# lab-emi/CleanUMamba

Measured on AMD Instinct MI355X. Metric: audio samples/sec/node (train step, E8, 10s@16kHz), higher is better.
Workload: dtype f16; 1 GPU; CleanUMamba-E8 (41.4M) full train step: fwd + L1 + multi-res STFT loss + bwd + grad all-reduce + clip + Adam; 10 s @ 16 kHz clips; global_batch=16, batch_per_gpu=16, clip_samples=160000, parallelism=dp1, weights=random init (reference init, seed 0)

## Files before the change

cleanumamba_amd/csrc/dec7.hip:

```cpp
#include "outer_common.h"

namespace cum {

constexpr int D7_H = 64;
constexpr int D7_J = 128;
constexpr int D7_R = 32;
constexpr int D7_ZS = 288;
constexpr int D7_US = 144;
constexpr int D7_SLAB = D7_J * D7_H + D7_J + D7_H * 4 + 2;

struct Dec7FwdParams {
  const void *u;
  const void *w1p;
  const float *b1p;
  const float *wt;
  const float *bt;
  void *out;
  int64_t M;
  int pitch, valid;
  int64_t zero_tail;
  int steps_per_wg;
};

template <typename T>
__global__ __launch_bounds__(256) void dec7_fwd_kernel(const Dec7FwdParams p) {
  static_assert(sizeof(T) == 2, "16-bit element types only");
  __shared__ __attribute__((aligned(16))) unsigned char ut_all[2][D7_R * D7_US];
  __shared__ float4 pv_all[2][4][D7_R];
  __shared__ float carry[2][2];

  const int tid = threadIdx.x, lane = tid & 63;
  const int w = uniform(tid >> 6);
  const int g = lane >> 4, r = lane & 15;
  const T *u = static_cast<const T *>(p.u) + D7_H;
  T *out = static_cast<T *>(p.out) + 8;
  if (blockIdx.x == 0) {
    if (tid < 8) out[tid - 8] = (T)0.f;
    for (int64_t i = tid; i < p.zero_tail; i += 256) out[2 * p.M * 8 + i] = (T)0.f;
  }
// ... 82 lines not shown
        }
      }
      if (row == 0) {
        prv[2] = carry[par ^ 1][0];
        prv[3] = carry[par ^ 1][1];
      }
      if (row == D7_R - 1) carry[par][q] = cur[2 + q];
      const int64_t m = m0 + row;
      if (s >= s_begin && m < p.M) {
        const bool ok = e0_row_ok(t0, row, m0, p.M, (unsigned)p.pitch, (unsigned)p.valid + 1u);
        const float v = ok ? cur[q] + prv[2 + q] + btv : 0.f;
        *reinterpret_cast<uint4 *>(out + (2 * m + q) * 8) = make_uint4(e0_pack2<T>(v, 0.f), 0u, 0u, 0u);
      }
    }
  }
}

struct Dec7BwdParams {
  const void *u;
  const void *dy;
  const unsigned char *mask;
  const void *w1p;
  const float *b1p;
  const float *wt;
  void *du;
  void *dpre;
  float *slabs;
  int64_t M;
  int pitch, valid;
  int64_t zero_tail;
};

template <typename T>
__global__ __launch_bounds__(256) void dec7_bwd_kernel(const Dec7BwdParams p) {
  static_assert(sizeof(T) == 2, "16-bit element types only");
  constexpr int BUF = D7_R * D7_US + D7_R * D7_ZS + 2 * D7_R * D7_US + 320 + 512;
  __shared__ __attribute__((aligned(16))) unsigned char lds[2 * BUF];

  const int tid = threadIdx.x, lane = tid & 63;
  const int w = uniform(tid >> 6);
  const int g = lane >> 4, r = lane & 15;
  const T *u = static_cast<const T *>(p.u) + D7_H;
  const T *dy = static_cast<const T *>(p.dy);
  T *du = static_cast<T *>(p.du) + D7_H, *dpre = static_cast<T *>(p.dpre) + D7_H;
  if (blockIdx.x == 0) {
    for (int i = tid; i < D7_H; i += 256) du[i - D7_H] = dpre[i - D7_H] = (T)0.f;
    for (int64_t i = tid; i < p.zero_tail; i += 256) du[p.M * D7_H + i] = dpre[p.M * D7_H + i] = (T)0.f;
  }
  e0_u32x4 wA[2][2], wB[4];
  float ba[4], bb[4], wtr[4][4];
  {
    const T *w1 = static_cast<const T *>(p.w1p);
#pragma unroll
    for (int jt = 0; jt < 2; ++jt)
#pragma unroll
      for (int ks = 0; ks < 2; ++ks)
        wA[jt][ks] = *reinterpret_cast<const e0_u32x4 *>(w1 + (int64_t)(32 * w + 16 * jt + r) * D7_H + 32 * ks + 8 * g);
#pragma unroll
    for (int ks = 0; ks < 4; ++ks) {
      unsigned v[4];
#pragma unroll
      for (int q = 0; q < 4; ++q) {
        const int j = 32 * ks + 8 * g + 2 * q;
        const unsigned short lo = __builtin_bit_cast(unsigned short, w1[(int64_t)j * D7_H + 16 * w + r]);
        const unsigned short hi = __builtin_bit_cast(unsigned short, w1[(int64_t)(j + 1) * D7_H + 16 * w + r]);
        v[q] = (unsigned)lo | ((unsigned)hi << 16);
      }
      wB[ks] = e0_u32x4{v[0], v[1], v[2], v[3]};
    }
#pragma unroll
    for (int rr = 0; rr < 4; ++rr) {
      ba[rr] = p.b1p[32 * w + 4 * g + rr];
      bb[rr] = p.b1p[32 * w + 16 + 4 * g + rr];
#pragma unroll
      for (int k = 0; k < 4; ++k) wtr[rr][k] = (float)(T)p.wt[(16 * w + 4 * g + rr) * 4 + k];
    }
  }
  const unsigned one2 = __is_same(T, f16) ? 0x3C003C00u : 0x3F803F80u;
  const e0_u32x4 ones = e0_u32x4{one2, one2, one2, one2};

  e0_f32x4 acc1[2][4];
  e0_f32x4 accb[2];
#pragma unroll
  for (int it = 0; it < 2; ++it) {
    accb[it] = e0_f32x4{0.f, 0.f, 0.f, 0.f};
#pragma unroll
    for (int nt = 0; nt < 4; ++nt) acc1[it][nt] = e0_f32x4{0.f, 0.f, 0.f, 0.f};
  }
  float awt[4][4];
#pragma unroll
  for (int rr = 0; rr < 4; ++rr)
#pragma unroll
    for (int k = 0; k < 4; ++k) awt[rr][k] = 0.f;
  float sdy = 0.f;

  const int64_t nsteps = (p.M + D7_R - 1) / D7_R;
  constexpr int PF = 3;
  uint4 uc[PF];
  float xs[PF];
  unsigned mk[PF];
  auto fetch = [&](int64_t s, uint4 &c, float &x, unsigned &mw) {
    const int64_t m0 = s * D7_R;
    int64_t m = m0 + (tid >> 3);
    m = m < p.M ? m : p.M - 1;
    c = *reinterpret_cast<const uint4 *>(u + m * D7_H + (tid & 7) * 8);
    x = 0.f;
    if (tid < 72) {
      int64_t row = 1 + 2 * m0 + tid;
      const int64_t last = 2 * p.M + 2;
      row = row < last ? row : last;
      x = (float)dy[row * 8];
    }
    mw = 0u;
    if (tid >= 128) {
      int64_t mm = m0 + ((tid - 128) >> 2);
      mm = mm < p.M ? mm : p.M - 1;
      mw = *reinterpret_cast<const unsigned *>(p.mask + mm * 16 + (tid & 3) * 4);
    }
  };
  int64_t s = blockIdx.x;
#pragma unroll
  for (int i = 0; i < PF; ++i) {
    const int64_t sf = s + (int64_t)i * gridDim.x;
    fetch(sf < nsteps ? sf : nsteps - 1, uc[i], xs[i], mk[i]);
  }
  int par = 0;
  for (; s < nsteps; s += gridDim.x, par ^= 1) {
    unsigned char *ut = lds + par * BUF, *zt = ut + D7_R * D7_US, *dut = zt + D7_R * D7_ZS, *dpt = dut + D7_R * D7_US;
    float *xt = reinterpret_cast<float *>(dpt + D7_R * D7_US);
    unsigned *mt_ = reinterpret_cast<unsigned *>(xt + 80);
    const int64_t m0 = s * D7_R;
    const unsigned t0 = (unsigned)uniform((int)((unsigned)m0 % (unsigned)p.pitch));
    *reinterpret_cast<uint4 *>(ut + (tid >> 3) * D7_US + (tid & 7) * 16) = uc[0];
    if (tid < 72) xt[tid] = 2 * m0 + tid < 2 * p.M ? xs[0] : 0.f;
    if (tid >= 128) mt_[tid - 128] = mk[0];
    __syncthreads();
    {
#pragma unroll
      for (int i = 0; i + 1 < PF; ++i) {
        uc[i] = uc[i + 1];
        xs[i] = xs[i + 1];
        mk[i] = mk[i + 1];
      }
      const int64_t sf = s + (int64_t)PF * gridDim.x;
      if (sf < nsteps) fetch(sf, uc[PF - 1], xs[PF - 1], mk[PF - 1]);
    }
    if (w == 0) sdy += xt[lane];
#pragma unroll
    for (int mt = 0; mt < 2; ++mt) {
      e0_f32x4 da = e0_f32x4{0.f, 0.f, 0.f, 0.f}, db = da;
#pragma unroll
      for (int ks = 0; ks < 2; ++ks) {
        const e0_u32x4 ub = *reinterpret_cast<const e0_u32x4 *>(ut + (16 * mt + r) * D7_US + (4 * ks + g) * 16);
        da = e0_mfma<T>(wA[0][ks], ub, da);
        db = e0_mfma<T>(wA[1][ks], ub, db);
      }
      const int row = 16 * mt + r;
      const bool ok = e0_row_ok(t0, row, m0, p.M, (unsigned)p.pitch, (unsigned)p.valid);
      const float d0 = xt[2 * row], d1 = xt[2 * row + 1], d2 = xt[2 * row + 2], d3 = xt[2 * row + 3];
      float za[4], zb[4];
#pragma unroll
      for (int rr = 0; rr < 4; ++rr) {
        const float sg = sigmoidf_(db[rr] + bb[rr]);
        const float gv = e0_keep(ok, (float)(T)((da[rr] + ba[rr]) * sg));
        float dg = d0 * wtr[rr][0];
        dg = fmaf(d1, wtr[rr][1], dg);
        dg = fmaf(d2, wtr[rr][2], dg);
        dg = fmaf(d3, wtr[rr][3], dg);
        za[rr] = e0_keep(ok, dg * sg);
        zb[rr] = dg * gv * (1.f - sg);
        awt[rr][0] = fmaf(gv, d0, awt[rr][0]);
        awt[rr][1] = fmaf(gv, d1, awt[rr][1]);
        awt[rr][2] = fmaf(gv, d2, awt[rr][2]);
        awt[rr][3] = fmaf(gv, d3, awt[rr][3]);
      }
      *reinterpret_cast<uint2 *>(zt + row * D7_ZS + (32 * w + 4 * g) * 2) = make_uint2(e0_pack2<T>(za[0], za[1]), e0_pack2<T>(za[2], za[3]));
      *reinterpret_cast<uint2 *>(zt + row * D7_ZS + (32 * w + 16 + 4 * g) * 2) = make_uint2(e0_pack2<T>(zb[0], zb[1]), e0_pack2<T>(zb[2], zb[3]));
    }
    __syncthreads();
    {
      e0_f32x4 d1[2] = {e0_f32x4{0.f, 0.f, 0.f, 0.f}, e0_f32x4{0.f, 0.f, 0.f, 0.f}};
#pragma unroll
      for (int mt = 0; mt < 2; ++mt)
#pragma unroll
        for (int ks = 0; ks < 4; ++ks) {
          const e0_u32x4 a = *reinterpret_cast<const e0_u32x4 *>(zt + (16 * mt + r) * D7_ZS + (4 * ks + g) * 16);
          d1[mt] = e0_mfma<T>(a, wB[ks], d1[mt]);
        }
      const int h = 16 * w + r;
#pragma unroll
      for (int mt = 0; mt < 2; ++mt)
#pragma unroll
        for (int rr = 0; rr < 4; ++rr) {
          const int row = 16 * mt + 4 * g + rr;
          const unsigned bit = (reinterpret_cast<const unsigned char *>(mt_)[row * 16 + (h >> 2)] >> (h & 3)) & 1u;
          const T v = (T)d1[mt][rr];
          *reinterpret_cast<T *>(dut + row * D7_US + h * 2) = v;
          *reinterpret_cast<T *>(dpt + row * D7_US + h * 2) = bit ? v : (T)0.f;
        }
    }
    {
      const int q = r >> 2, pp = r & 3;
      e0_u32x4 af[2], bf[4];
#pragma unroll
      for (int it = 0; it < 2; ++it) af[it] = e0_tr_read<D7_ZS>(zt + (8 * g + q) * D7_ZS + (32 * w + 16 * it + 4 * pp) * 2);
#pragma unroll
      for (int nt = 0; nt < 4; ++nt) bf[nt] = e0_tr_read<D7_US>(ut + (8 * g + q) * D7_US + (16 * nt + 4 * pp) * 2);
#pragma unroll
      for (int it = 0; it < 2; ++it) {
#pragma unroll
        for (int nt = 0; nt < 4; ++nt) acc1[it][nt] = e0_mfma<T>(af[it], bf[nt], acc1[it][nt]);
        accb[it] = e0_mfma<T>(af[it], ones, accb[it]);
      }
    }
    __syncthreads();
    {
      const int row = tid >> 3, ch = tid & 7;
      const int64_t m = m0 + row;
      if (m < p.M) {
        *reinterpret_cast<uint4 *>(du + m * D7_H + ch * 8) = *reinterpret_cast<const uint4 *>(dut + row * D7_US + ch * 16);
        *reinterpret_cast<uint4 *>(dpre + m * D7_H + ch * 8) = *reinterpret_cast<const uint4 *>(dpt + row * D7_US + ch * 16);
      }
    }
  }

  float *slab = p.slabs + (int64_t)blockIdx.x * D7_SLAB;
#pragma unroll
  for (int it = 0; it < 2; ++it)
#pragma unroll
    for (int rr = 0; rr < 4; ++rr) {
      const int j = 32 * w + 16 * it + 4 * g + rr;
#pragma unroll
      for (int nt = 0; nt < 4; ++nt) slab[j * D7_H + 16 * nt + r] = acc1[it][nt][rr];
      if (r == 0) slab[D7_J * D7_H + j] = accb[it][rr];
    }
  float *s1 = slab + D7_J * D7_H + D7_J;
#pragma unroll
  for (int rr = 0; rr < 4; ++rr)
#pragma unroll
    for (int k = 0; k < 4; ++k) {
      const float v = row16_allsum(awt[rr][k]);
      if (r == 0) s1[(16 * w + 4 * g + rr) * 4 + k] = v;
    }
  if (w == 0) {
    sdy += __shfl_xor(sdy, 2, 64);
    sdy += __shfl_xor(sdy, 4, 64);
    sdy += __shfl_xor(sdy, 8, 64);
    sdy += __shfl_xor(sdy, 16, 64);
    sdy += __shfl_xor(sdy, 32, 64);
    if (lane < 2) s1[D7_H * 4 + lane] = sdy;
// ... 46 lines not shown
}

using namespace cum;

static int dec7_fwd_workgroups(int64_t M) {
  const int64_t steps = (M + D7_R - 1) / D7_R;
  return (int)(steps < 1024 ? steps : 1024);
}

extern "C" int cum_dec7_fwd(int32_t dtype, int64_t M, int32_t pitch, int32_t valid, const void *u, const void *w1p,
                            const float *b1p, const float *wt, const float *bt, void *out, int64_t zero_tail, void *stream) {
  CUM_REQUIRE(is16(dtype), "dec7_fwd: 16-bit element types only (f32 takes the generic path)");
  CUM_REQUIRE(M > 0 && M < 1073741823LL && pitch >= 32 && valid > 0 && valid < pitch && zero_tail >= 0, "dec7_fwd: bad geometry");
  CUM_REQUIRE(u && w1p && b1p && wt && bt && out, "dec7_fwd: null tensor");
  CUM_REQUIRE(((uintptr_t)u & 15) == 0 && ((uintptr_t)out & 15) == 0 && ((uintptr_t)w1p & 15) == 0,
              "dec7_fwd: u, out and w1p must be 16-byte aligned");
  hipStream_t st = (hipStream_t)stream;
  Dec7FwdParams p{};
  p.u = u; p.w1p = w1p; p.b1p = b1p; p.wt = wt; p.bt = bt; p.out = out; p.M = M; p.pitch = pitch; p.valid = valid;
  p.zero_tail = zero_tail;
  const int64_t steps = (M + D7_R - 1) / D7_R;
  int nwg = dec7_fwd_workgroups(M);
  p.steps_per_wg = (int)((steps + nwg - 1) / nwg);
  nwg = (int)((steps + p.steps_per_wg - 1) / p.steps_per_wg);
  if (dtype == CUM_F16)
    hipLaunchKernelGGL(dec7_fwd_kernel<f16>, dim3(nwg), dim3(256), 0, st, p);
  else
    hipLaunchKernelGGL(dec7_fwd_kernel<__bf16>, dim3(nwg), dim3(256), 0, st, p);
  CUM_CHECK_LAUNCH();
  return CUM_OK;
}

extern "C" int32_t cum_dec7_bwd_workgroups(int64_t M) {
  const int64_t steps = (M + D7_R - 1) / D7_R;
  return (int32_t)(steps < 1 ? 1 : (steps > 512 ? 512 : steps));
}

extern "C" int64_t cum_dec7_bwd_workspace_elems(int64_t M) {
  return ((int64_t)cum_dec7_bwd_workgroups(M) + D7_RG) * D7_SLAB;
}

extern "C" int cum_dec7_bwd(int32_t dtype, int64_t M, int32_t pitch, int32_t valid, const void *dY, const void *u,
                            const void *mask, const void *w1p, const float *b1p, const float *wt, void *dU, void *dpre,
                            int64_t zero_tail, float *slot_w1, float *slot_wt, float *workspace, void *stream) {
  CUM_REQUIRE(is16(dtype), "dec7_bwd: 16-bit element types only (f32 takes the generic path)");
  CUM_REQUIRE(M > 0 && M < 1073741823LL && pitch >= 32 && valid > 0 && valid < pitch && zero_tail >= 0, "dec7_bwd: bad geometry");
  CUM_REQUIRE(dY && u && mask && w1p && b1p && wt && dU && dpre && slot_w1 && slot_wt && workspace, "dec7_bwd: null tensor");
  CUM_REQUIRE(((uintptr_t)u & 15) == 0 && ((uintptr_t)dU & 15) == 0 && ((uintptr_t)dpre & 15) == 0 && ((uintptr_t)w1p & 15) == 0 &&
                  ((uintptr_t)mask & 3) == 0, "dec7_bwd: u, dU, dpre and w1p must be 16-byte aligned, mask 4-byte aligned");
  hipStream_t st = (hipStream_t)stream;
  Dec7BwdParams p{};
  p.u = u; p.dy = dY; p.mask = static_cast<const unsigned char *>(mask); p.w1p = w1p; p.b1p = b1p; p.wt = wt; p.du = dU;
  p.dpre = dpre; p.slabs = workspace; p.M = M; p.pitch = pitch; p.valid = valid; p.zero_tail = zero_tail;
  const int nwg = cum_dec7_bwd_workgroups(M);
  if (dtype == CUM_F16)
    hipLaunchKernelGGL(dec7_bwd_kernel<f16>, dim3(nwg), dim3(256), 0, st, p);
  else
    hipLaunchKernelGGL(dec7_bwd_kernel<__bf16>, dim3(nwg), dim3(256), 0, st, p);
  CUM_CHECK_LAUNCH();
  float *part = workspace + (int64_t)nwg * D7_SLAB;
  hipLaunchKernelGGL(dec7_bwd_reduce1_kernel, dim3((D7_SLAB + 255) / 256, D7_RG), dim3(256), 0, st, workspace, nwg, part);
  constexpr int nout = D7_J * D7_H + D7_J + 16 * 128 + 16;
  hipLaunchKernelGGL(dec7_bwd_reduce2_kernel, dim3((nout + 255) / 256), dim3(256), 0, st, part, slot_w1, slot_wt);
  CUM_CHECK_LAUNCH();
  return CUM_OK;
}
```

cleanumamba_amd/csrc/enc0.hip:

```cpp
#include "outer_common.h"

namespace cum {

constexpr int E0_H = 64;
constexpr int E0_J = 128;
constexpr int E0_R = 32;
constexpr int E0_ZS = 288;
constexpr int E0_YS = 144;
constexpr int E0_SLAB = E0_J * E0_H + E0_J + E0_H * 4 + E0_H;

struct Enc0BwdParams {
  const void *dz;
  const void *xin;
  const float *w1;
  const float *b1;
  const void *w2p;
  float *slabs;
  int64_t M;
  int pitch, valid;
};

template <typename T>
__global__ __launch_bounds__(256) void enc0_bwd_kernel(const Enc0BwdParams p) {
  static_assert(sizeof(T) == 2, "16-bit element types only");
// ... 16 lines not shown
  }
  e0_u32x4 wB[4];
  {
    const T *w2 = static_cast<const T *>(p.w2p);
#pragma unroll
    for (int ks = 0; ks < 4; ++ks) {
      unsigned v[4];
#pragma unroll
      for (int q = 0; q < 4; ++q) {
        const int j = 32 * ks + 8 * g + 2 * q;
        const unsigned short lo = __builtin_bit_cast(unsigned short, w2[(int64_t)j * E0_H + 16 * w + r]);
        const unsigned short hi = __builtin_bit_cast(unsigned short, w2[(int64_t)(j + 1) * E0_H + 16 * w + r]);
        v[q] = (unsigned)lo | ((unsigned)hi << 16);
      }
      wB[ks] = e0_u32x4{v[0], v[1], v[2], v[3]};
    }
  }
  const unsigned one2 = __is_same(T, f16) ? 0x3C003C00u : 0x3F803F80u;
  const e0_u32x4 ones = e0_u32x4{one2, one2, one2, one2};

  e0_f32x4 acc2[2][4];
  e0_f32x4 accb[2];
#pragma unroll
  for (int it = 0; it < 2; ++it) {
    accb[it] = e0_f32x4{0.f, 0.f, 0.f, 0.f};
#pragma unroll
    for (int nt = 0; nt < 4; ++nt) acc2[it][nt] = e0_f32x4{0.f, 0.f, 0.f, 0.f};
  }
  float a1[4] = {0.f, 0.f, 0.f, 0.f}, ab1 = 0.f;

  const int64_t nsteps = (p.M + E0_R - 1) / E0_R;
  constexpr int PF = 3;
  uint4 zc[PF][2];
  float xs[PF];
  auto fetch = [&](int64_t s, uint4 (&z)[2], float &x) {
    const int64_t m0 = s * E0_R;
#pragma unroll
    for (int it = 0; it < 2; ++it) {
      const int c = tid + 256 * it;
      int64_t m = m0 + (c >> 4);
      m = m < p.M ? m : p.M - 1;
      z[it] = *reinterpret_cast<const uint4 *>(dz + m * E0_J + (c & 15) * 8);
    }
    x = 0.f;
    if (tid < 72) {
      int64_t row = 1 + 2 * m0 + tid;
      const int64_t last = 2 * p.M + 2;
      row = row < last ? row : last;
      x = (float)xin[row * 8];
    }
  };
  int64_t s = blockIdx.x;
#pragma unroll
  for (int i = 0; i < PF; ++i) {
    const int64_t sf = s + (int64_t)i * gridDim.x;
    fetch(sf < nsteps ? sf : nsteps - 1, zc[i], xs[i]);
  }
  int par = 0;
  for (; s < nsteps; s += gridDim.x, par ^= 1) {
    unsigned char *zt = lds + par * BUF, *yt = zt + E0_R * E0_ZS;
    float *xt = reinterpret_cast<float *>(yt + E0_R * E0_YS);
    const int64_t m0 = s * E0_R;
    const unsigned t0 = (unsigned)uniform((int)((unsigned)m0 % (unsigned)p.pitch));
#pragma unroll
    for (int it = 0; it < 2; ++it) {
      const int c = tid + 256 * it;
      const bool ok = e0_row_ok(t0, c >> 4, m0, p.M, (unsigned)p.pitch, (unsigned)p.valid);
      *reinterpret_cast<uint4 *>(zt + (c >> 4) * E0_ZS + (c & 15) * 16) = ok ? zc[0][it] : make_uint4(0, 0, 0, 0);
    }
    if (tid < 72) xt[tid] = xs[0];
    __syncthreads();
    {
      const bool ok = e0_row_ok(t0, yrow, m0, p.M, (unsigned)p.pitch, (unsigned)p.valid);
      const float x0 = xt[2 * yrow], x1 = xt[2 * yrow + 1], x2 = xt[2 * yrow + 2], x3 = xt[2 * yrow + 3];
      float y[8];
#pragma unroll
      for (int e = 0; e < 8; ++e) {
        float v = b1r[e];
        v = fmaf(w1r[e][0], x0, v);
        v = fmaf(w1r[e][1], x1, v);
        v = fmaf(w1r[e][2], x2, v);
        v = fmaf(w1r[e][3], x3, v);
        y[e] = ok && v > 0.f ? v : 0.f;
      }
      const uint4 pk = make_uint4(e0_pack2<T>(y[0], y[1]), e0_pack2<T>(y[2], y[3]), e0_pack2<T>(y[4], y[5]), e0_pack2<T>(y[6], y[7]));
      *reinterpret_cast<uint4 *>(yt + yrow * E0_YS + yh0 * 2) = pk;
    }
    __syncthreads();
    {
#pragma unroll
      for (int i = 0; i + 1 < PF; ++i) {
        zc[i][0] = zc[i + 1][0];
        zc[i][1] = zc[i + 1][1];
        xs[i] = xs[i + 1];
      }
      const int64_t sf = s + (int64_t)PF * gridDim.x;
      if (sf < nsteps) fetch(sf, zc[PF - 1], xs[PF - 1]);
    }

    e0_f32x4 d1[2] = {e0_f32x4{0.f, 0.f, 0.f, 0.f}, e0_f32x4{0.f, 0.f, 0.f, 0.f}};
#pragma unroll
    for (int mt = 0; mt < 2; ++mt)
#pragma unroll
      for (int ks = 0; ks < 4; ++ks) {
        const e0_u32x4 a = *reinterpret_cast<const e0_u32x4 *>(zt + (16 * mt + r) * E0_ZS + (4 * ks + g) * 16);
        d1[mt] = e0_mfma<T>(a, wB[ks], d1[mt]);
      }
#pragma unroll
    for (int mt = 0; mt < 2; ++mt)
#pragma unroll
      for (int rr = 0; rr < 4; ++rr) {
        const int row = 16 * mt + 4 * g + rr;
        const unsigned short yv = *reinterpret_cast<const unsigned short *>(yt + row * E0_YS + (16 * w + r) * 2);
        const float dv = (yv & 0x7FFFu) != 0 ? d1[mt][rr] : 0.f;
        ab1 += dv;
        a1[0] = fmaf(dv, xt[2 * row], a1[0]);
        a1[1] = fmaf(dv, xt[2 * row + 1], a1[1]);
        a1[2] = fmaf(dv, xt[2 * row + 2], a1[2]);
        a1[3] = fmaf(dv, xt[2 * row + 3], a1[3]);
      }
    const int q = r >> 2, pp = r & 3;
    e0_u32x4 af[2], bf[4];
#pragma unroll
    for (int it = 0; it < 2; ++it) {
      const unsigned char *a0 = zt + (8 * g + q) * E0_ZS + (32 * w + 16 * it + 4 * pp) * 2;
      e0_u32x2 lo, hi;
      asm volatile("ds_read_b64_tr_b16 %0, %1" : "=v"(lo) : "v"((unsigned)(uintptr_t)(__attribute__((address_space(3))) void *)a0) : "memory");
      asm volatile("ds_read_b64_tr_b16 %0, %1 offset:%2" : "=v"(hi) : "v"((unsigned)(uintptr_t)(__attribute__((address_space(3))) void *)a0), "n"(4 * E0_ZS) : "memory");
      asm volatile("s_waitcnt lgkmcnt(0)" : "+v"(lo), "+v"(hi) : : "memory");
      af[it] = e0_u32x4{lo.x, lo.y, hi.x, hi.y};
    }
#pragma unroll
    for (int nt = 0; nt < 4; ++nt) {
      const unsigned char *b0 = yt + (8 * g + q) * E0_YS + (16 * nt + 4 * pp) * 2;
      e0_u32x2 lo, hi;
      asm volatile("ds_read_b64_tr_b16 %0, %1" : "=v"(lo) : "v"((unsigned)(uintptr_t)(__attribute__((address_space(3))) void *)b0) : "memory");
      asm volatile("ds_read_b64_tr_b16 %0, %1 offset:%2" : "=v"(hi) : "v"((unsigned)(uintptr_t)(__attribute__((address_space(3))) void *)b0), "n"(4 * E0_YS) : "memory");
      asm volatile("s_waitcnt lgkmcnt(0)" : "+v"(lo), "+v"(hi) : : "memory");
      bf[nt] = e0_u32x4{lo.x, lo.y, hi.x, hi.y};
    }
#pragma unroll
    for (int it = 0; it < 2; ++it) {
#pragma unroll
      for (int nt = 0; nt < 4; ++nt) acc2[it][nt] = e0_mfma<T>(af[it], bf[nt], acc2[it][nt]);
      accb[it] = e0_mfma<T>(af[it], ones, accb[it]);
    }
  }

  float *slab = p.slabs + (int64_t)blockIdx.x * E0_SLAB;
#pragma unroll
  for (int it = 0; it < 2; ++it)
#pragma unroll
    for (int rr = 0; rr < 4; ++rr) {
      const int j = 32 * w + 16 * it + 4 * g + rr;
#pragma unroll
      for (int nt = 0; nt < 4; ++nt) slab[j * E0_H + 16 * nt + r] = acc2[it][nt][rr];
      if (r == 0) slab[E0_J * E0_H + j] = accb[it][rr];
    }
#pragma unroll
  for (int k = 0; k < 4; ++k) {
    a1[k] += __shfl_xor(a1[k], 16, 64);
    a1[k] += __shfl_xor(a1[k], 32, 64);
  }
  ab1 += __shfl_xor(ab1, 16, 64);
  ab1 += __shfl_xor(ab1, 32, 64);
  if (g == 0) {
    const int h = 16 * w + r;
    float *s1 = slab + E0_J * E0_H + E0_J;
#pragma unroll
    for (int k = 0; k < 4; ++k) s1[h * 4 + k] = a1[k];
    s1[E0_H * 4 + h] = ab1;
  }
// ... 59 lines not shown
  const int g = lane >> 4, r = lane & 15;
  const T *xin = static_cast<const T *>(p.xin);
  T *out = static_cast<T *>(p.out) + E0_H;
  T *gate = static_cast<T *>(p.gate);
  if (blockIdx.x == 0) {
    for (int i = tid; i < E0_H; i += 256) out[i - E0_H] = (T)0.f;
    for (int64_t i = tid; i < p.zero_tail; i += 256) out[p.M * E0_H + i] = (T)0.f;
  }
  const int yrow = lane & 31, yh0 = 16 * w + 8 * (lane >> 5);
  float w1r[8][4], b1r[8];
#pragma unroll
  for (int e = 0; e < 8; ++e) {
#pragma unroll
    for (int k = 0; k < 4; ++k) w1r[e][k] = (float)(T)p.w1[(yh0 + e) * 4 + k];
    b1r[e] = p.b1[yh0 + e];
  }
  e0_u32x4 wA[2][2];
  float ba[4], bb[4];
  {
    const T *w2 = static_cast<const T *>(p.w2p);
#pragma unroll
    for (int jt = 0; jt < 2; ++jt)
#pragma unroll
      for (int ks = 0; ks < 2; ++ks)
        wA[jt][ks] = *reinterpret_cast<const e0_u32x4 *>(w2 + (int64_t)(32 * w + 16 * jt + r) * E0_H + 32 * ks + 8 * g);
#pragma unroll
    for (int rr = 0; rr < 4; ++rr) {
      ba[rr] = p.b2p[32 * w + 4 * g + rr];
      bb[rr] = p.b2p[32 * w + 16 + 4 * g + rr];
    }
  }
  const int64_t nsteps = (p.M + E0_R - 1) / E0_R;
  constexpr int PF = 4;
  float xs[PF];
  auto fetch = [&](int64_t s, float &x) {
    x = 0.f;
    if (tid < 72) {
      int64_t row = 1 + 2 * s * E0_R + tid;
      const int64_t last = 2 * p.M + 2;
      row = row < last ? row : last;
      x = (float)xin[row * 8];
    }
  };
  int64_t s = blockIdx.x;
#pragma unroll
  for (int i = 0; i < PF; ++i) {
    const int64_t sf = s + (int64_t)i * gridDim.x;
    fetch(sf < nsteps ? sf : nsteps - 1, xs[i]);
  }
  int par = 0;
  for (; s < nsteps; s += gridDim.x, par ^= 1) {
    unsigned char *yt = lds + par * BUF, *ot = yt + E0_R * E0_YS, *gt = ot + E0_R * E0_YS;
    float *xt = reinterpret_cast<float *>(gt + E0_R * E0_YS);
    const int64_t m0 = s * E0_R;
    const unsigned t0 = (unsigned)uniform((int)((unsigned)m0 % (unsigned)p.pitch));
    if (tid < 72) xt[tid] = xs[0];
    __syncthreads();
    {
#pragma unroll
      for (int i = 0; i + 1 < PF; ++i) xs[i] = xs[i + 1];
      const int64_t sf = s + (int64_t)PF * gridDim.x;
      if (sf < nsteps) fetch(sf, xs[PF - 1]);
    }
    {
      const bool ok = e0_row_ok(t0, yrow, m0, p.M, (unsigned)p.pitch, (unsigned)p.valid);
      const float x0 = xt[2 * yrow], x1 = xt[2 * yrow + 1], x2 = xt[2 * yrow + 2], x3 = xt[2 * yrow + 3];
      float y[8];
#pragma unroll
      for (int e = 0; e < 8; ++e) {
        float v = b1r[e];
        v = fmaf(w1r[e][0], x0, v);
        v = fmaf(w1r[e][1], x1, v);
        v = fmaf(w1r[e][2], x2, v);
        v = fmaf(w1r[e][3], x3, v);
        y[e] = ok && v > 0.f ? v : 0.f;
      }
      *reinterpret_cast<uint4 *>(yt + yrow * E0_YS + yh0 * 2) =
          make_uint4(e0_pack2<T>(y[0], y[1]), e0_pack2<T>(y[2], y[3]), e0_pack2<T>(y[4], y[5]), e0_pack2<T>(y[6], y[7]));
    }
    __syncthreads();
#pragma unroll
    for (int mt = 0; mt < 2; ++mt) {
      e0_f32x4 da = e0_f32x4{0.f, 0.f, 0.f, 0.f}, db = da;
#pragma unroll
      for (int ks = 0; ks < 2; ++ks) {
        const e0_u32x4 yb = *reinterpret_cast<const e0_u32x4 *>(yt + (16 * mt + r) * E0_YS + (4 * ks + g) * 16);
        da = e0_mfma<T>(wA[0][ks], yb, da);
        db = e0_mfma<T>(wA[1][ks], yb, db);
      }
      const bool ok = e0_row_ok(t0, 16 * mt + r, m0, p.M, (unsigned)p.pitch, (unsigned)p.valid);
      float o[4], gv[4];
#pragma unroll
      for (int rr = 0; rr < 4; ++rr) {
        const float a = da[rr] + ba[rr], b = db[rr] + bb[rr];
        o[rr] = e0_keep(ok, a * sigmoidf_(b));
        gv[rr] = ok ? b : 0.f;
      }
      const int off = (16 * mt + r) * E0_YS + (16 * w + 4 * g) * 2;
      *reinterpret_cast<uint2 *>(ot + off) = make_uint2(e0_pack2<T>(o[0], o[1]), e0_pack2<T>(o[2], o[3]));
      *reinterpret_cast<uint2 *>(gt + off) = make_uint2(e0_pack2<T>(gv[0], gv[1]), e0_pack2<T>(gv[2], gv[3]));
    }
    __syncthreads();
    {
      const int row = tid >> 3, ch = tid & 7;
      const int64_t m = m0 + row;
      if (m < p.M) {
        *reinterpret_cast<uint4 *>(out + m * E0_H + ch * 8) = *reinterpret_cast<const uint4 *>(ot + row * E0_YS + ch * 16);
        if (gate) *reinterpret_cast<uint4 *>(gate + m * E0_H + ch * 8) = *reinterpret_cast<const uint4 *>(gt + row * E0_YS + ch * 16);
      }
    }
  }
}

}

using namespace cum;

extern "C" int cum_enc0_fwd(int32_t dtype, int64_t M, int32_t pitch, int32_t valid, const void *xin, const float *w1,
                            const float *b1, const void *w2p, const float *b2p, void *out, int64_t zero_tail, void *gate,
                            void *stream) {
  CUM_REQUIRE(is16(dtype), "enc0_fwd: 16-bit element types only (f32 takes the generic path)");
  CUM_REQUIRE(M > 0 && M < 2147483647LL && pitch > 0 && valid > 0 && valid <= pitch && zero_tail >= 0, "enc0_fwd: bad geometry");
  CUM_REQUIRE(xin && w1 && b1 && w2p && b2p && out, "enc0_fwd: null tensor");
  CUM_REQUIRE(((uintptr_t)out & 15) == 0 && ((uintptr_t)gate & 15) == 0 && ((uintptr_t)w2p & 15) == 0,
              "enc0_fwd: out, gate and w2p must be 16-byte aligned");
  hipStream_t st = (hipStream_t)stream;
  Enc0FwdParams p{};
  p.xin = xin; p.w1 = w1; p.b1 = b1; p.w2p = w2p; p.b2p = b2p; p.out = out; p.gate = gate; p.M = M; p.pitch = pitch;
  p.valid = valid; p.zero_tail = zero_tail;
  const int64_t steps = (M + E0_R - 1) / E0_R;
  const int nwg = (int)(steps < 1024 ? steps : 1024);
  if (dtype == CUM_F16)
    hipLaunchKernelGGL(enc0_fwd_kernel<f16>, dim3(nwg), dim3(256), 0, st, p);
  else
    hipLaunchKernelGGL(enc0_fwd_kernel<__bf16>, dim3(nwg), dim3(256), 0, st, p);
  CUM_CHECK_LAUNCH();
  return CUM_OK;
}

extern "C" int32_t cum_enc0_bwd_workgroups(int64_t M) {
  const int64_t steps = (M + E0_R - 1) / E0_R;
  return (int32_t)(steps < 1 ? 1 : (steps > 512 ? 512 : steps));
}

extern "C" int64_t cum_enc0_bwd_workspace_elems(int64_t M) {
  return ((int64_t)cum_enc0_bwd_workgroups(M) + E0_RG) * E0_SLAB;
}

extern "C" int cum_enc0_bwd(int32_t dtype, int64_t M, int32_t pitch, int32_t valid, const void *dZ, const void *xin,
                            const float *w1, const float *b1, const void *w2p, float *slot_w2, float *slot_w1,
                            float *workspace, void *stream) {
  CUM_REQUIRE(is16(dtype), "enc0_bwd: 16-bit element types only (f32 takes the generic path)");
  CUM_REQUIRE(M > 0 && M < 2147483647LL && pitch > 0 && valid > 0 && valid <= pitch, "enc0_bwd: bad geometry");
  CUM_REQUIRE(dZ && xin && w1 && b1 && w2p && slot_w2 && slot_w1 && workspace, "enc0_bwd: null tensor");
  CUM_REQUIRE(((uintptr_t)dZ & 15) == 0, "enc0_bwd: dZ must be 16-byte aligned");
  hipStream_t st = (hipStream_t)stream;
  Enc0BwdParams p{};
  p.dz = dZ; p.xin = xin; p.w1 = w1; p.b1 = b1; p.w2p = w2p; p.slabs = workspace; p.M = M; p.pitch = pitch; p.valid = valid;
  const int nwg = cum_enc0_bwd_workgroups(M);
  if (dtype == CUM_F16)
    hipLaunchKernelGGL(enc0_bwd_kernel<f16>, dim3(nwg), dim3(256), 0, st, p);
  else
    hipLaunchKernelGGL(enc0_bwd_kernel<__bf16>, dim3(nwg), dim3(256), 0, st, p);
  CUM_CHECK_LAUNCH();
  float *part = workspace + (int64_t)nwg * E0_SLAB;
  hipLaunchKernelGGL(enc0_bwd_reduce1_kernel, dim3((E0_SLAB + 255) / 256, E0_RG), dim3(256), 0, st, workspace, nwg, part);
  hipLaunchKernelGGL(enc0_bwd_reduce2_kernel, dim3((E0_SLAB + 255) / 256), dim3(256), 0, st, part, slot_w2, slot_w1);
  CUM_CHECK_LAUNCH();
  return CUM_OK;
}
```

cleanumamba_amd/csrc/outer_common.h:

```cpp
#pragma once
#include "common.h"

namespace cum {

typedef __attribute__((ext_vector_type(8))) __bf16 e0_bf16x8;
typedef __attribute__((ext_vector_type(8))) _Float16 e0_f16x8;
typedef __attribute__((ext_vector_type(4))) float e0_f32x4;
typedef __attribute__((ext_vector_type(4))) unsigned e0_u32x4;
typedef __attribute__((ext_vector_type(2))) unsigned e0_u32x2;

template <typename T>
__device__ __forceinline__ e0_f32x4 e0_mfma(e0_u32x4 a, e0_u32x4 b, e0_f32x4 c) {
  if constexpr (__is_same(T, f16))
    return __builtin_amdgcn_mfma_f32_16x16x32_f16(__builtin_bit_cast(e0_f16x8, a), __builtin_bit_cast(e0_f16x8, b), c, 0, 0, 0);
  else
    return __builtin_amdgcn_mfma_f32_16x16x32_bf16(__builtin_bit_cast(e0_bf16x8, a), __builtin_bit_cast(e0_bf16x8, b), c, 0, 0, 0);
}

__device__ __forceinline__ bool e0_row_ok(unsigned t0, int row, int64_t m0, const int64_t M, unsigned pitch, unsigned valid) {
  unsigned tt = t0 + (unsigned)row;
  tt = tt >= pitch ? tt - pitch : tt;
  return m0 + row < M && tt < valid;
}

__device__ __forceinline__ float e0_keep(bool ok, float v) {
  asm volatile("" : "+v"(v));
  return ok ? v : 0.f;
}

template <typename T>
__device__ __forceinline__ unsigned e0_pack2(float a, float b) {
  typedef T V2 __attribute__((ext_vector_type(2)));
  V2 v = {(T)a, (T)b};
  return __builtin_bit_cast(unsigned, v);
}

template <int STRIDE>
__device__ __forceinline__ e0_u32x4 e0_tr_read(const unsigned char *a0) {
  e0_u32x2 lo, hi;
  const unsigned addr = (unsigned)(uintptr_t)(__attribute__((address_space(3))) void *)a0;
  asm volatile("ds_read_b64_tr_b16 %0, %1" : "=v"(lo) : "v"(addr) : "memory");
  asm volatile("ds_read_b64_tr_b16 %0, %1 offset:%2" : "=v"(hi) : "v"(addr), "n"(4 * STRIDE) : "memory");
  asm volatile("s_waitcnt lgkmcnt(0)" : "+v"(lo), "+v"(hi) : : "memory");
  return e0_u32x4{lo.x, lo.y, hi.x, hi.y};
}

}
```

cleanumamba_amd/network/convstack.py:

```python
import ctypes
import os

import numpy as np
import torch

from .. import hip


def rup(x, m):
    return (x + m - 1) // m * m


class Geo:

    def __init__(self, B, T, C):
        self.B, self.T, self.C = B, T, C
        self.P = T + 2
        self.Cp = rup(C, 8)
        self.M = B * self.P
        self.slack = 2 + (128 + self.Cp - 1) // self.Cp
        self.R = 1 + self.M + self.slack

    def new(self, dtype, device, zero=False):
        if zero:
# ... 938 lines not shown
    gemm(xbuf, 0, gi.Cp, wp, bp, ybuf, go.Cp, N, gi.M, gi.P, gi.T + 1, hip.EPI_RELU if relu else hip.EPI_BIAS, N,
         res=skip, r_off=go.Cp, ldr=N, aux=act, x_off=go.Cp, ldz=N, geo=go)
    return ybuf, (act if keep else (ybuf if relu else None))


def _glu_bwd(z, ybuf, dy, go):
    G = z.shape[1] // 16
    dz = torch.empty(go.M, G * 32, dtype=z.dtype, device=z.device)
    with torch.cuda.device(z.device):
        hip.check(hip.lib().cum_glu_bwd_gate(hip.dtype_code(z.dtype), go.M, G, go.Cp, hip.ptr(z), G * 16,
                                             hip.ptr(ybuf[1:]), go.Cp, hip.ptr(dy[1:]), go.Cp, hip.ptr(dz), G * 32,
                                             hip.stream_ptr()))
    return dz


def _glu_wgrad(dz, xbuf, gi, M, out):
    G32 = dz.shape[1]
    wgrad(dz, 0, G32, G32, xbuf, gi.Cp, gi.Cp, gi.Cp, M, out=out)


def _glu_dgrad_weights(w, gi, G32, dt):
    sh = tuple(w.shape)
    Nd, Kd = rup(gi.Cp, 16), rup(G32, bk_of(dt))
    return take(w, ("glu_dgrad", sh, Nd, Kd),
                lambda: torch.nn.functional.pad(lay_glu_fwd(sh, G32, Nd).t(), (0, Kd - G32)), dt)


_ENC_BITS = os.environ.get("CUM_ENC_BITS", "1") != "0"
_ENC0_FUSED = os.environ.get("CUM_ENC0_FUSED", "1") != "0"


def _enc0_ok(w1, w2, gi, gm, go, dt):
    return (_ENC0_FUSED and dt in hip.HALF_TYPES and tuple(w1.shape) == (64, 1, 4) and tuple(w2.shape) == (128, 64, 1)
            and gi.C == 1 and gi.Cp == 8 and gm.C == 64 and go.C == 64 and w1.dtype == torch.float32)


def _enc0_w2p(w2, gm, dt):
    sh = tuple(w2.shape)
    G = (sh[0] // 2 + 15) // 16
    Kp = rup(gm.Cp, bk_of(dt))
    wp = take(w2, ("glu_fwd", sh, G * 32, Kp), lambda: lay_glu_fwd(sh, G * 32, Kp), dt)
    return wp


def _enc0_fwd(xbuf, w1, b1, w2, b2, gm, go, save_z):
    dt, dev = xbuf.dtype, xbuf.device
    wp = _enc0_w2p(w2, gm, dt)
    bp = take(b2, ("glu_vec", w2.shape[0]), lambda: lay_glu_vec(w2.shape[0]), torch.float32)
    ybuf = go.new(dt, dev)
    z = torch.empty(go.M, 64, dtype=dt, device=dev) if save_z else None
    with torch.cuda.device(dev):
        hip.check(hip.lib().cum_enc0_fwd(hip.dtype_code(dt), go.M, go.P, go.T, hip.ptr(xbuf), hip.ptr(w1.detach()),
                                         hip.ptr(b1.detach()), hip.ptr(wp), hip.ptr(bp), hip.ptr(ybuf), go.tail, hip.ptr(z),
                                         hip.stream_ptr()))
    return ybuf, z


_ENCH_FUSED = os.environ.get("CUM_ENCH_FUSED", "1") != "0"


def _ench_ok(w1, w2, gi, gm, go, dt):
    return (_ENCH_FUSED and dt in hip.HALF_TYPES and tuple(w1.shape) == (128, 64, 4) and tuple(w2.shape) == (256, 128, 1)
            and gi.Cp == 64 and gm.Cp == 128 and go.Cp == 128 and gm.P >= 3)


def _ench_fwd(xbuf, w1, b1, w2, b2, gi, gm, go, save_z):
    dt, dev = xbuf.dtype, xbuf.device
# ... 339 lines not shown
```

Baseline: 129.5 million audio samples/s.

## Double dec7 backward step rows, batch transposed LDS reads, defer sample conversion

```diff
diff --git a/cleanumamba_amd/csrc/dec7.hip b/cleanumamba_amd/csrc/dec7.hip
--- a/cleanumamba_amd/csrc/dec7.hip
+++ b/cleanumamba_amd/csrc/dec7.hip
@@ -5,6 +5,7 @@
 constexpr int D7_H = 64;
 constexpr int D7_J = 128;
 constexpr int D7_R = 32;
+constexpr int D7_RB = 64;
 constexpr int D7_ZS = 288;
 constexpr int D7_US = 144;
 constexpr int D7_SLAB = D7_J * D7_H + D7_J + D7_H * 4 + 2;
@@ -153,10 +154,10 @@
 };
 
 template <typename T>
-__global__ __launch_bounds__(256) void dec7_bwd_kernel(const Dec7BwdParams p) {
+__global__ __launch_bounds__(256, 2) void dec7_bwd_kernel(const Dec7BwdParams p) {
   static_assert(sizeof(T) == 2, "16-bit element types only");
-  constexpr int BUF = D7_R * D7_US + D7_R * D7_ZS + 2 * D7_R * D7_US + 320 + 512;
-  __shared__ __attribute__((aligned(16))) unsigned char lds[2 * BUF];
+  constexpr int BUF = D7_RB * D7_US + D7_RB * D7_ZS + 544 + 1024;
+  __shared__ __attribute__((aligned(16))) unsigned char lds[2 * BUF + 2 * D7_RB * D7_US];
 
   const int tid = threadIdx.x, lane = tid & 63;
   const int w = uniform(tid >> 6);
@@ -215,26 +216,28 @@
     for (int k = 0; k < 4; ++k) awt[rr][k] = 0.f;
   float sdy = 0.f;
 
-  const int64_t nsteps = (p.M + D7_R - 1) / D7_R;
-  constexpr int PF = 3;
-  uint4 uc[PF];
-  float xs[PF];
+  const int64_t nsteps = (p.M + D7_RB - 1) / D7_RB;
+  constexpr int PF = 2;
+  uint4 uc[PF][2];
+  unsigned xs[PF];
   unsigned mk[PF];
-  auto fetch = [&](int64_t s, uint4 &c, float &x, unsigned &mw) {
-    const int64_t m0 = s * D7_R;
-    int64_t m = m0 + (tid >> 3);
-    m = m < p.M ? m : p.M - 1;
-    c = *reinterpret_cast<const uint4 *>(u + m * D7_H + (tid & 7) * 8);
-    x = 0.f;
-    if (tid < 72) {
+  auto fetch = [&](int64_t s, uint4 (&c)[2], unsigned &x, unsigned &mw) {
+    const int64_t m0 = s * D7_RB;
+#pragma unroll
+    for (int it = 0; it < 2; ++it) {
+      int64_t m = m0 + (tid >> 3) + 32 * it;
+      m = m < p.M ? m : p.M - 1;
+      c[it] = *reinterpret_cast<const uint4 *>(u + m * D7_H + (tid & 7) * 8);
+    }
+    x = 0u;
+    if (tid < 136) {
       int64_t row = 1 + 2 * m0 + tid;
       const int64_t last = 2 * p.M + 2;
       row = row < last ? row : last;
-      x = (float)dy[row * 8];
-    }
-    mw = 0u;
-    if (tid >= 128) {
-      int64_t mm = m0 + ((tid - 128) >> 2);
+      x = reinterpret_cast<const unsigned short *>(dy)[row * 8];
+    }
+    {
+      int64_t mm = m0 + (tid >> 2);
       mm = mm < p.M ? mm : p.M - 1;
       mw = *reinterpret_cast<const unsigned *>(p.mask + mm * 16 + (tid & 3) * 4);
     }
@@ -247,28 +250,31 @@
   }
   int par = 0;
   for (; s < nsteps; s += gridDim.x, par ^= 1) {
-    unsigned char *ut = lds + par * BUF, *zt = ut + D7_R * D7_US, *dut = zt + D7_R * D7_ZS, *dpt = dut + D7_R * D7_US;
-    float *xt = reinterpret_cast<float *>(dpt + D7_R * D7_US);
-    unsigned *mt_ = reinterpret_cast<unsigned *>(xt + 80);
-    const int64_t m0 = s * D7_R;
+    unsigned char *ut = lds + par * BUF, *zt = ut + D7_RB * D7_US, *dut = lds + 2 * BUF, *dpt = dut + D7_RB * D7_US;
+    float *xt = reinterpret_cast<float *>(zt + D7_RB * D7_ZS);
+    unsigned *mt_ = reinterpret_cast<unsigned *>(xt + 136);
+    const int64_t m0 = s * D7_RB;
     const unsigned t0 = (unsigned)uniform((int)((unsigned)m0 % (unsigned)p.pitch));
-    *reinterpret_cast<uint4 *>(ut + (tid >> 3) * D7_US + (tid & 7) * 16) = uc[0];
-    if (tid < 72) xt[tid] = 2 * m0 + tid < 2 * p.M ? xs[0] : 0.f;
-    if (tid >= 128) mt_[tid - 128] = mk[0];
+#pragma unroll
+    for (int it = 0; it < 2; ++it)
+      *reinterpret_cast<uint4 *>(ut + ((tid >> 3) + 32 * it) * D7_US + (tid & 7) * 16) = uc[0][it];
+    if (tid < 136) xt[tid] = 2 * m0 + tid < 2 * p.M ? e0_sample<T>(xs[0]) : 0.f;
+    mt_[tid] = mk[0];
     __syncthreads();
     {
 #pragma unroll
       for (int i = 0; i + 1 < PF; ++i) {
-        uc[i] = uc[i + 1];
+        uc[i][0] = uc[i + 1][0];
+        uc[i][1] = uc[i + 1][1];
         xs[i] = xs[i + 1];
         mk[i] = mk[i + 1];
       }
       const int64_t sf = s + (int64_t)PF * gridDim.x;
       if (sf < nsteps) fetch(sf, uc[PF - 1], xs[PF - 1], mk[PF - 1]);
     }
-    if (w == 0) sdy += xt[lane];
-#pragma unroll
-    for (int mt = 0; mt < 2; ++mt) {
+    if (w == 0) sdy += xt[lane] + xt[64 + lane];
+#pragma unroll
+    for (int mt = 0; mt < 4; ++mt) {
       e0_f32x4 da = e0_f32x4{0.f, 0.f, 0.f, 0.f}, db = da;
 #pragma unroll
       for (int ks = 0; ks < 2; ++ks) {
@@ -277,7 +283,7 @@
         db = e0_mfma<T>(wA[1][ks], ub, db);
       }
       const int row = 16 * mt + r;
-      const bool ok = e0_row_ok(t0, row, m0, p.M, (unsigned)p.pitch, (unsigned)p.valid);
+      const bool ok = e0_row_ok<D7_RB>(t0, row, m0, p.M, (unsigned)p.pitch, (unsigned)p.valid);
       const float d0 = xt[2 * row], d1 = xt[2 * row + 1], d2 = xt[2 * row + 2], d3 = xt[2 * row + 3];
       float za[4], zb[4];
 #pragma unroll
@@ -299,44 +305,47 @@
       *reinterpret_cast<uint2 *>(zt + row * D7_ZS + (32 * w + 16 + 4 * g) * 2) = make_uint2(e0_pack2<T>(zb[0], zb[1]), e0_pack2<T>(zb[2], zb[3]));
     }
     __syncthreads();
-    {
-      e0_f32x4 d1[2] = {e0_f32x4{0.f, 0.f, 0.f, 0.f}, e0_f32x4{0.f, 0.f, 0.f, 0.f}};
-#pragma unroll
-      for (int mt = 0; mt < 2; ++mt)
-#pragma unroll
-        for (int ks = 0; ks < 4; ++ks) {
-          const e0_u32x4 a = *reinterpret_cast<const e0_u32x4 *>(zt + (16 * mt + r) * D7_ZS + (4 * ks + g) * 16);
-          d1[mt] = e0_mfma<T>(a, wB[ks], d1[mt]);
-        }
-      const int h = 16 * w + r;
-#pragma unroll
-      for (int mt = 0; mt < 2; ++mt)
-#pragma unroll
-        for (int rr = 0; rr < 4; ++rr) {
-          const int row = 16 * mt + 4 * g + rr;
-          const unsigned bit = (reinterpret_cast<const unsigned char *>(mt_)[row * 16 + (h >> 2)] >> (h & 3)) & 1u;
-          const T v = (T)d1[mt][rr];
-          *reinterpret_cast<T *>(dut + row * D7_US + h * 2) = v;
-          *reinterpret_cast<T *>(dpt + row * D7_US + h * 2) = bit ? v : (T)0.f;
-        }
+#pragma unroll
+    for (int mt = 0; mt < 4; ++mt) {
+      e0_f32x4 d1 = e0_f32x4{0.f, 0.f, 0.f, 0.f};
+#pragma unroll
+      for (int ks = 0; ks < 4; ++ks) {
+        const e0_u32x4 zb = *reinterpret_cast<const e0_u32x4 *>(zt + (16 * mt + r) * D7_ZS + (4 * ks + g) * 16);
+        d1 = e0_mfma<T>(wB[ks], zb, d1);
+      }
+      const int row = 16 * mt + r;
+      const unsigned nib = reinterpret_cast<const unsigned char *>(mt_)[row * 16 + 4 * w + g];
+      const unsigned v01 = e0_pack2<T>(d1[0], d1[1]), v23 = e0_pack2<T>(d1[2], d1[3]);
+      const unsigned m01 = ((nib & 1u) ? 0xFFFFu : 0u) | ((nib & 2u) ? 0xFFFF0000u : 0u);
+      const unsigned m23 = ((nib & 4u) ? 0xFFFFu : 0u) | ((nib & 8u) ? 0xFFFF0000u : 0u);
+      *reinterpret_cast<uint2 *>(dut + row * D7_US + (16 * w + 4 * g) * 2) = make_uint2(v01, v23);
+      *reinterpret_cast<uint2 *>(dpt + row * D7_US + (16 * w + 4 * g) * 2) = make_uint2(v01 & m01, v23 & m23);
     }
     {
       const int q = r >> 2, pp = r & 3;
-      e0_u32x4 af[2], bf[4];
-#pragma unroll
-      for (int it = 0; it < 2; ++it) af[it] = e0_tr_read<D7_ZS>(zt + (8 * g + q) * D7_ZS + (32 * w + 16 * it + 4 * pp) * 2);
-#pragma unroll
-      for (int nt = 0; nt < 4; ++nt) bf[nt] = e0_tr_read<D7_US>(ut + (8 * g + q) * D7_US + (16 * nt + 4 * pp) * 2);
-#pragma unroll
-      for (int it = 0; it < 2; ++it) {
-#pragma unroll
-        for (int nt = 0; nt < 4; ++nt) acc1[it][nt] = e0_mfma<T>(af[it], bf[nt], acc1[it][nt]);
-        accb[it] = e0_mfma<T>(af[it], ones, accb[it]);
+      const unsigned za = e0_lds_addr(zt + (8 * g + q) * D7_ZS + (32 * w + 4 * pp) * 2);
+      const unsigned ua = e0_lds_addr(ut + (8 * g + q) * D7_US + (4 * pp) * 2);
+#pragma unroll
+      for (int kh = 0; kh < 2; ++kh) {
+        e0_u32x2 lo[6], hi[6];
+        if (kh == 0) e0_tr_issue6<D7_ZS, D7_US, 0>(za, ua, lo, hi);
+        else e0_tr_issue6<D7_ZS, D7_US, 32>(za, ua, lo, hi);
+        e0_tr_wait6(lo, hi);
+        e0_u32x4 f[6];
+#pragma unroll
+        for (int i = 0; i < 6; ++i) f[i] = __builtin_shufflevector(lo[i], hi[i], 0, 1, 2, 3);
+#pragma unroll
+        for (int it = 0; it < 2; ++it) {
+#pragma unroll
+          for (int nt = 0; nt < 4; ++nt) acc1[it][nt] = e0_mfma<T>(f[it], f[2 + nt], acc1[it][nt]);
+          accb[it] = e0_mfma<T>(f[it], ones, accb[it]);
+        }
       }
     }
     __syncthreads();
-    {
-      const int row = tid >> 3, ch = tid & 7;
+#pragma unroll
+    for (int it = 0; it < 2; ++it) {
+      const int row = (tid >> 3) + 32 * it, ch = tid & 7;
       const int64_t m = m0 + row;
       if (m < p.M) {
         *reinterpret_cast<uint4 *>(du + m * D7_H + ch * 8) = *reinterpret_cast<const uint4 *>(dut + row * D7_US + ch * 16);
@@ -449,7 +458,7 @@
 }
 
 extern "C" int32_t cum_dec7_bwd_workgroups(int64_t M) {
-  const int64_t steps = (M + D7_R - 1) / D7_R;
+  const int64_t steps = (M + D7_RB - 1) / D7_RB;
   return (int32_t)(steps < 1 ? 1 : (steps > 512 ? 512 : steps));
 }
 
diff --git a/cleanumamba_amd/csrc/enc0.hip b/cleanumamba_amd/csrc/enc0.hip
--- a/cleanumamba_amd/csrc/enc0.hip
+++ b/cleanumamba_amd/csrc/enc0.hip
@@ -72,8 +72,8 @@
   const int64_t nsteps = (p.M + E0_R - 1) / E0_R;
   constexpr int PF = 3;
   uint4 zc[PF][2];
-  float xs[PF];
-  auto fetch = [&](int64_t s, uint4 (&z)[2], float &x) {
+  unsigned xs[PF];
+  auto fetch = [&](int64_t s, uint4 (&z)[2], unsigned &x) {
     const int64_t m0 = s * E0_R;
 #pragma unroll
     for (int it = 0; it < 2; ++it) {
@@ -82,12 +82,12 @@
       m = m < p.M ? m : p.M - 1;
       z[it] = *reinterpret_cast<const uint4 *>(dz + m * E0_J + (c & 15) * 8);
     }
-    x = 0.f;
+    x = 0u;
     if (tid < 72) {
       int64_t row = 1 + 2 * m0 + tid;
       const int64_t last = 2 * p.M + 2;
       row = row < last ? row : last;
-      x = (float)xin[row * 8];
+      x = reinterpret_cast<const unsigned short *>(xin)[row * 8];
     }
   };
   int64_t s = blockIdx.x;
@@ -108,7 +108,7 @@
       const bool ok = e0_row_ok(t0, c >> 4, m0, p.M, (unsigned)p.pitch, (unsigned)p.valid);
       *reinterpret_cast<uint4 *>(zt + (c >> 4) * E0_ZS + (c & 15) * 16) = ok ? zc[0][it] : make_uint4(0, 0, 0, 0);
     }
-    if (tid < 72) xt[tid] = xs[0];
+    if (tid < 72) xt[tid] = e0_sample<T>(xs[0]);
     __syncthreads();
     {
       const bool ok = e0_row_ok(t0, yrow, m0, p.M, (unsigned)p.pitch, (unsigned)p.valid);
@@ -161,23 +161,15 @@
       }
     const int q = r >> 2, pp = r & 3;
     e0_u32x4 af[2], bf[4];
-#pragma unroll
-    for (int it = 0; it < 2; ++it) {
-      const unsigned char *a0 = zt + (8 * g + q) * E0_ZS + (32 * w + 16 * it + 4 * pp) * 2;
-      e0_u32x2 lo, hi;
-      asm volatile("ds_read_b64_tr_b16 %0, %1" : "=v"(lo) : "v"((unsigned)(uintptr_t)(__attribute__((address_space(3))) void *)a0) : "memory");
-      asm volatile("ds_read_b64_tr_b16 %0, %1 offset:%2" : "=v"(hi) : "v"((unsigned)(uintptr_t)(__attribute__((address_space(3))) void *)a0), "n"(4 * E0_ZS) : "memory");
-      asm volatile("s_waitcnt lgkmcnt(0)" : "+v"(lo), "+v"(hi) : : "memory");
-      af[it] = e0_u32x4{lo.x, lo.y, hi.x, hi.y};
-    }
-#pragma unroll
-    for (int nt = 0; nt < 4; ++nt) {
-      const unsigned char *b0 = yt + (8 * g + q) * E0_YS + (16 * nt + 4 * pp) * 2;
-      e0_u32x2 lo, hi;
-      asm volatile("ds_read_b64_tr_b16 %0, %1" : "=v"(lo) : "v"((unsigned)(uintptr_t)(__attribute__((address_space(3))) void *)b0) : "memory");
-      asm volatile("ds_read_b64_tr_b16 %0, %1 offset:%2" : "=v"(hi) : "v"((unsigned)(uintptr_t)(__attribute__((address_space(3))) void *)b0), "n"(4 * E0_YS) : "memory");
-      asm volatile("s_waitcnt lgkmcnt(0)" : "+v"(lo), "+v"(hi) : : "memory");
-      bf[nt] = e0_u32x4{lo.x, lo.y, hi.x, hi.y};
+    {
+      e0_u32x2 lo[6], hi[6];
+      e0_tr_issue6<E0_ZS, E0_YS, 0>(e0_lds_addr(zt + (8 * g + q) * E0_ZS + (32 * w + 4 * pp) * 2),
+                                    e0_lds_addr(yt + (8 * g + q) * E0_YS + (4 * pp) * 2), lo, hi);
+      e0_tr_wait6(lo, hi);
+#pragma unroll
+      for (int it = 0; it < 2; ++it) af[it] = __builtin_shufflevector(lo[it], hi[it], 0, 1, 2, 3);
+#pragma unroll
+      for (int nt = 0; nt < 4; ++nt) bf[nt] = __builtin_shufflevector(lo[2 + nt], hi[2 + nt], 0, 1, 2, 3);
     }
 #pragma unroll
     for (int it = 0; it < 2; ++it) {
@@ -303,14 +295,14 @@
   }
   const int64_t nsteps = (p.M + E0_R - 1) / E0_R;
   constexpr int PF = 4;
-  float xs[PF];
-  auto fetch = [&](int64_t s, float &x) {
-    x = 0.f;
+  unsigned xs[PF];
+  auto fetch = [&](int64_t s, unsigned &x) {
+    x = 0u;
     if (tid < 72) {
       int64_t row = 1 + 2 * s * E0_R + tid;
       const int64_t last = 2 * p.M + 2;
       row = row < last ? row : last;
-      x = (float)xin[row * 8];
+      x = reinterpret_cast<const unsigned short *>(xin)[row * 8];
     }
   };
   int64_t s = blockIdx.x;
@@ -325,7 +317,7 @@
     float *xt = reinterpret_cast<float *>(gt + E0_R * E0_YS);
     const int64_t m0 = s * E0_R;
     const unsigned t0 = (unsigned)uniform((int)((unsigned)m0 % (unsigned)p.pitch));
-    if (tid < 72) xt[tid] = xs[0];
+    if (tid < 72) xt[tid] = e0_sample<T>(xs[0]);
     __syncthreads();
     {
 #pragma unroll
@@ -391,7 +383,7 @@
                             const float *b1, const void *w2p, const float *b2p, void *out, int64_t zero_tail, void *gate,
                             void *stream) {
   CUM_REQUIRE(is16(dtype), "enc0_fwd: 16-bit element types only (f32 takes the generic path)");
-  CUM_REQUIRE(M > 0 && M < 2147483647LL && pitch > 0 && valid > 0 && valid <= pitch && zero_tail >= 0, "enc0_fwd: bad geometry");
+  CUM_REQUIRE(M > 0 && M < 2147483647LL && pitch >= 32 && valid > 0 && valid <= pitch && zero_tail >= 0, "enc0_fwd: bad geometry");
   CUM_REQUIRE(xin && w1 && b1 && w2p && b2p && out, "enc0_fwd: null tensor");
   CUM_REQUIRE(((uintptr_t)out & 15) == 0 && ((uintptr_t)gate & 15) == 0 && ((uintptr_t)w2p & 15) == 0,
               "enc0_fwd: out, gate and w2p must be 16-byte aligned");
@@ -422,7 +414,7 @@
                             const float *w1, const float *b1, const void *w2p, float *slot_w2, float *slot_w1,
                             float *workspace, void *stream) {
   CUM_REQUIRE(is16(dtype), "enc0_bwd: 16-bit element types only (f32 takes the generic path)");
-  CUM_REQUIRE(M > 0 && M < 2147483647LL && pitch > 0 && valid > 0 && valid <= pitch, "enc0_bwd: bad geometry");
+  CUM_REQUIRE(M > 0 && M < 2147483647LL && pitch >= 32 && valid > 0 && valid <= pitch, "enc0_bwd: bad geometry");
   CUM_REQUIRE(dZ && xin && w1 && b1 && w2p && slot_w2 && slot_w1 && workspace, "enc0_bwd: null tensor");
   CUM_REQUIRE(((uintptr_t)dZ & 15) == 0, "enc0_bwd: dZ must be 16-byte aligned");
   hipStream_t st = (hipStream_t)stream;
diff --git a/cleanumamba_amd/csrc/outer_common.h b/cleanumamba_amd/csrc/outer_common.h
--- a/cleanumamba_amd/csrc/outer_common.h
+++ b/cleanumamba_amd/csrc/outer_common.h
@@ -17,9 +17,12 @@
     return __builtin_amdgcn_mfma_f32_16x16x32_bf16(__builtin_bit_cast(e0_bf16x8, a), __builtin_bit_cast(e0_bf16x8, b), c, 0, 0, 0);
 }
 
+template <int R = 32>
 __device__ __forceinline__ bool e0_row_ok(unsigned t0, int row, int64_t m0, const int64_t M, unsigned pitch, unsigned valid) {
+  static_assert(R % 32 == 0, "one conditional subtraction per 32 rows of the step");
   unsigned tt = t0 + (unsigned)row;
-  tt = tt >= pitch ? tt - pitch : tt;
+#pragma unroll
+  for (int i = 0; i < R / 32; ++i) tt = tt >= pitch ? tt - pitch : tt;
   return m0 + row < M && tt < valid;
 }
 
@@ -35,14 +38,38 @@
   return __builtin_bit_cast(unsigned, v);
 }
 
-template <int STRIDE>
-__device__ __forceinline__ e0_u32x4 e0_tr_read(const unsigned char *a0) {
-  e0_u32x2 lo, hi;
-  const unsigned addr = (unsigned)(uintptr_t)(__attribute__((address_space(3))) void *)a0;
-  asm volatile("ds_read_b64_tr_b16 %0, %1" : "=v"(lo) : "v"(addr) : "memory");
-  asm volatile("ds_read_b64_tr_b16 %0, %1 offset:%2" : "=v"(hi) : "v"(addr), "n"(4 * STRIDE) : "memory");
-  asm volatile("s_waitcnt lgkmcnt(0)" : "+v"(lo), "+v"(hi) : : "memory");
-  return e0_u32x4{lo.x, lo.y, hi.x, hi.y};
+template <typename T>
+__device__ __forceinline__ float e0_sample(unsigned raw) {
+  return (float)__builtin_bit_cast(T, (unsigned short)raw);
+}
+
+template <int STRIDE, int OFF>
+__device__ __forceinline__ void e0_tr_issue(unsigned addr, e0_u32x2 &lo, e0_u32x2 &hi) {
+  static_assert(OFF >= 0 && OFF + 4 * STRIDE < 65536, "ds offset field: 16 bits");
+  asm volatile("ds_read_b64_tr_b16 %0, %1 offset:%2" : "=v"(lo) : "v"(addr), "n"(OFF) : "memory");
+  asm volatile("ds_read_b64_tr_b16 %0, %1 offset:%2" : "=v"(hi) : "v"(addr), "n"(OFF + 4 * STRIDE) : "memory");
+}
+
+template <int ZS, int YS, int ROW0>
+__device__ __forceinline__ void e0_tr_issue6(unsigned za, unsigned ya, e0_u32x2 (&lo)[6], e0_u32x2 (&hi)[6]) {
+  e0_tr_issue<ZS, ROW0 * ZS>(za, lo[0], hi[0]);
+  e0_tr_issue<ZS, ROW0 * ZS + 32>(za, lo[1], hi[1]);
+  e0_tr_issue<YS, ROW0 * YS>(ya, lo[2], hi[2]);
+  e0_tr_issue<YS, ROW0 * YS + 32>(ya, lo[3], hi[3]);
+  e0_tr_issue<YS, ROW0 * YS + 64>(ya, lo[4], hi[4]);
+  e0_tr_issue<YS, ROW0 * YS + 96>(ya, lo[5], hi[5]);
+}
+
+__device__ __forceinline__ void e0_tr_wait6(e0_u32x2 (&lo)[6], e0_u32x2 (&hi)[6]) {
+  asm volatile("s_waitcnt lgkmcnt(0)"
+               : "+v"(lo[0]), "+v"(lo[1]), "+v"(lo[2]), "+v"(lo[3]), "+v"(lo[4]), "+v"(lo[5]), "+v"(hi[0]), "+v"(hi[1]),
+                 "+v"(hi[2]), "+v"(hi[3]), "+v"(hi[4]), "+v"(hi[5])
+               :
+               : "memory");
+}
+
+__device__ __forceinline__ unsigned e0_lds_addr(const unsigned char *p) {
+  return (unsigned)(uintptr_t)(__attribute__((address_space(3))) void *)p;
 }
 
 }
diff --git a/cleanumamba_amd/network/convstack.py b/cleanumamba_amd/network/convstack.py
--- a/cleanumamba_amd/network/convstack.py
+++ b/cleanumamba_amd/network/convstack.py
@@ -994,7 +994,7 @@
 
 def _enc0_ok(w1, w2, gi, gm, go, dt):
     return (_ENC0_FUSED and dt in hip.HALF_TYPES and tuple(w1.shape) == (64, 1, 4) and tuple(w2.shape) == (128, 64, 1)
-            and gi.C == 1 and gi.Cp == 8 and gm.C == 64 and go.C == 64 and w1.dtype == torch.float32)
+            and gi.C == 1 and gi.Cp == 8 and gm.C == 64 and go.C == 64 and go.P >= 32 and w1.dtype == torch.float32)
 
 
 def _enc0_w2p(w2, gm, dt):
```

Result: no change. 130.7 million audio samples/s, median of 6 (+0.9%).
